# tqch/ddpm-torch

Measured on AMD Instinct MI355X. Metric: training imgs/s/GPU + 1000-step DDPM samples/s, CIFAR-10 UNet @1/2/4/8 MI355X, higher is better.
Workload: dtype bf16; 1 GPU; configs/cifar10.json UNet (35.7M params), full Trainer.step, B=128 per GPU, 32x32, T=1000, dropout 0.1, Adam+clip+EMA; global_batch=128, rccl_ranks=1, parallelism=dp1

## Files before the change

ddpm-torch_amd/csrc/build.py:

```python
import glob
import os
import subprocess
import sys

HERE = os.path.dirname(os.path.abspath(__file__))
SOURCES = ["gemm.hip", "wgrad.hip", "wgrad1x1.hip", "attention.hip", "attention_stream.hip", "pointwise.hip", "conv3x3.hip", "edgeconv.hip", "norm.hip", "elementwise.hip", "optim.hip", "probe.hip", "plan.hip", "toymlp.hip", "manifold.hip", "batch.hip", "ddim.hip", "guidance.hip"]
OUT = os.path.join(HERE, "libddpm_hip.so")
FLAGS = ["--offload-arch=gfx950", "-O3", "-std=c++17", "-munsafe-fp-atomics", "-fPIC"]


def _stale(target, deps):
    if not os.path.exists(target):
        return True
    t = os.path.getmtime(target)
    return any(os.path.getmtime(d) > t for d in deps)


def build(force=False, verbose=True):
    hipcc = os.environ.get("HIPCC", "/opt/rocm/bin/hipcc")
    hdrs = sorted(glob.glob(os.path.join(HERE, "*.h")))
    inc = os.path.join(HERE, "..", "..", "include")
    abi = [os.path.join(inc, "ddpm_hip.h"), os.path.join(inc, "ddpm_hip_debug.h")]
    objs = []
    procs = []
    for s in SOURCES:
        src, obj = os.path.join(HERE, s), os.path.join(HERE, s.replace(".hip", ".o"))
        objs.append(obj)
        if force or _stale(obj, [src, *hdrs, *abi]):
            cmd = [hipcc, *FLAGS, "-c", src, "-o", obj]
            if verbose:
                print(" ".join(cmd), flush=True)
            procs.append((cmd, subprocess.Popen(cmd)))
    for cmd, p in procs:
        if p.wait() != 0:
            raise RuntimeError("hipcc failed: " + " ".join(cmd))
    if force or procs or _stale(OUT, objs):
        cmd = [hipcc, "--offload-arch=gfx950", "-shared", "-fPIC", "-o", OUT, *objs]
        if verbose:
            print(" ".join(cmd), flush=True)
        subprocess.check_call(cmd)
    return OUT


if __name__ == "__main__":
    print(build(force="--force" in sys.argv))
```

ddpm-torch_amd/csrc/pointwise.hip:

```cpp
#include "common.h"
#include <string.h>
#include <stdlib.h>

namespace {

typedef float f32x4v __attribute__((ext_vector_type(4)));
typedef unsigned u32x2 __attribute__((ext_vector_type(2)));

struct PwArgs {
    const bf16_t* x; long long x_ld; unsigned x_extent;
    const bf16_t* w; unsigned w_extent;
    bf16_t* out; long long out_ld;
    const float* bias;
    const bf16_t* res; long long res_ld;
    int accumulate;
    int M, N, K, tiles_m, tiles_n, ksteps;
    int spread;
};

template <int TM, int TN>
__global__ __launch_bounds__(512, 2)
void pw_conv_kernel(PwArgs a) {
    constexpr int WN = TN / 64, WM = 8 / WN;
    constexpr int MJ = TM / (32 * WM);
    constexpr int XV = TM / 64;
    constexpr int WV = TN / 64;
    constexpr int PER = XV + WV;
    constexpr int RING = TM + TN == 256 ? 4 : 3;
    constexpr int XB = TM * 128, WB = TN * 128, STAGE = XB + WB;
    static_assert(TN == 128 || TN == 256, "channel tile");
    constexpr int BIAS_AT = RING * STAGE;
    static_assert(BIAS_AT + 4096 <= 160 * 1024, "LDS");
    extern __shared__ __attribute__((aligned(16))) char smem[];
    const int tid = threadIdx.x, lane = tid & 63;
    const int wave = __builtin_amdgcn_readfirstlane(tid >> 6);
    const int wn = wave / WM, wm = wave % WM;

    const __amdgpu_buffer_rsrc_t rx = buffer_rsrc(a.x, a.x_extent), rw = buffer_rsrc(a.w, a.w_extent);
    const __amdgpu_buffer_rsrc_t rb = buffer_rsrc(a.bias ? (const void*)a.bias : (const void*)a.w, a.bias ? (unsigned)(a.N * 4) : 0u);

    unsigned xoff[4], woff[4];
#pragma unroll
    for (int i = 0; i < XV; ++i) {
        const int v = tid + 512 * i, row = v >> 3, lc = (v & 7) ^ ((row >> 1) & 7);
        xoff[i] = (unsigned)(((long long)row * a.x_ld + lc * 8) * 2);
    }
#pragma unroll
    for (int i = 0; i < WV; ++i) {
        const int v = tid + 512 * i, row = v >> 3, lc = (v & 7) ^ ((row >> 1) & 7);
        woff[i] = (unsigned)(((long long)row * a.K + lc * 8) * 2);
    }
    const unsigned x_tile_bytes = (unsigned)((long long)TM * a.x_ld * 2), w_tile_bytes = (unsigned)((long long)TN * a.K * 2);

    const int units = a.spread ? a.tiles_m * a.tiles_n : a.tiles_m;
    const int my_units = units > (int)blockIdx.x ? (units - 1 - (int)blockIdx.x) / (int)gridDim.x + 1 : 0;
    const int total = my_units * (a.spread ? 1 : a.tiles_n) * a.ksteps;
    const int mt0 = a.spread ? (int)blockIdx.x / a.tiles_n : (int)blockIdx.x, nt0 = a.spread ? (int)blockIdx.x - mt0 * a.tiles_n : 0;
    int i_vt = blockIdx.x, i_mt = mt0, i_nt = nt0, i_ks = 0, i_q = 0, i_tile = 0;
    auto issue = [&]() {
        char* dst = smem + (i_q % RING) * STAGE;
        if (i_ks == 0) {
            if (wave == 0 && a.bias)
                LDS_DMA16(rb, smem + BIAS_AT + (i_tile & 3) * 1024, lane < TN / 4 ? (unsigned)((i_nt * TN + lane * 4) * 4) : BUF_OOB, 0);
            ++i_tile;
        }
        const unsigned xb = (unsigned)i_mt * x_tile_bytes + (unsigned)(i_ks * 128);
        const unsigned wb = (unsigned)i_nt * w_tile_bytes + (unsigned)(i_ks * 128);
#pragma unroll
        for (int i = 0; i < XV; ++i)
            LDS_DMA16(rx, dst + (wave * 64 + 512 * i) * 16, xb + xoff[i], 0);
#pragma unroll
        for (int i = 0; i < WV; ++i)
            LDS_DMA16(rw, dst + XB + (wave * 64 + 512 * i) * 16, wb + woff[i], 0);
        ++i_q;
        if (++i_ks == a.ksteps) {
            i_ks = 0;
            if (a.spread) { i_vt += gridDim.x; i_mt = i_vt / a.tiles_n; i_nt = i_vt - i_mt * a.tiles_n; }
            else if (++i_nt == a.tiles_n) { i_nt = 0; i_mt += gridDim.x; }
        }
    };

    f32x16 acc[2][MJ];
#pragma unroll
    for (int i = 0; i < 2; ++i)
#pragma unroll
        for (int j = 0; j < MJ; ++j) acc[i][j] = (f32x16)(0.f);

#pragma unroll
    for (int t = 0; t < RING - 1; ++t)
        if (t < total) issue();

    const int sw = (lane >> 5) ^ ((lane >> 1) & 7);
    int c_vt = blockIdx.x, c_mt = mt0, c_nt = nt0, c_ks = 0, c_tile = 0;
    constexpr int ST = 4 * MJ;
    int st_window = 0;
    for (int q = 0; q < total; ++q) {
        const int newer = min(RING - 2, total - 1 - q);
        if (st_window > 0) {
            --st_window;
            if (newer >= 2) wait_vm<2 * PER + ST>(); else if (newer == 1) wait_vm<PER + ST>(); else wait_vm<ST>();
        } else {
            if (newer >= 2) wait_vm<2 * PER>(); else if (newer == 1) wait_vm<PER>(); else wait_vm<0>();
        }
        __builtin_amdgcn_s_barrier();
        const bool last = c_ks + 1 == a.ksteps;
        u32x2 rv[MJ][2][4], ov[MJ][2][4];
        const bool pre = last && (a.res || a.accumulate);
        if (pre) {
            const int n0 = c_nt * TN + wn * 64, p0 = c_mt * TM + wm * (32 * MJ);
#pragma unroll
            for (int j = 0; j < MJ; ++j)
#pragma unroll
                for (int i = 0; i < 2; ++i)
#pragma unroll
                    for (int g = 0; g < 4; ++g) {
                        const int p = p0 + j * 32 + (lane & 31), n = n0 + i * 32 + 8 * g + 4 * (lane >> 5);
                        const bool ok = p < a.M && n < a.N;
                        rv[j][i][g] = (u32x2)(0u); ov[j][i][g] = (u32x2)(0u);
                        if (ok && a.res) asm volatile("global_load_dwordx2 %0, %1, off" : "=v"(rv[j][i][g]) : "v"(a.res + (long long)p * a.res_ld + n) : "memory");
                        if (ok && a.accumulate) asm volatile("global_load_dwordx2 %0, %1, off" : "=v"(ov[j][i][g]) : "v"(a.out + (long long)p * a.out_ld + n) : "memory");
                    }
        }
        const bool issued = i_q < total, bias_rides = issued && i_ks == 0 && wave == 0 && a.bias;
        if (issued) issue();
        const char* xs = smem + (q % RING) * STAGE;
        const char* ws = xs + XB;
#pragma unroll
        for (int kc = 0; kc < 4; ++kc) {
            u32x4 fw[2], fx[MJ];
#pragma unroll
            for (int i = 0; i < 2; ++i) fw[i] = *reinterpret_cast<const u32x4*>(ws + (wn * 64 + i * 32 + (lane & 31)) * 128 + (((2 * kc) ^ sw) << 4));
#pragma unroll
            for (int j = 0; j < MJ; ++j) fx[j] = *reinterpret_cast<const u32x4*>(xs + (wm * (32 * MJ) + j * 32 + (lane & 31)) * 128 + (((2 * kc) ^ sw) << 4));
#pragma unroll
            for (int i = 0; i < 2; ++i)
#pragma unroll
                for (int j = 0; j < MJ; ++j)
                    acc[i][j] = __builtin_amdgcn_mfma_f32_32x32x16_bf16(__builtin_bit_cast(bf16x8, fw[i]), __builtin_bit_cast(bf16x8, fx[j]), acc[i][j], 0, 0, 0);
        }
        asm volatile("s_waitcnt lgkmcnt(0)" ::: "memory");
        if (pre) {
            if (!issued) wait_vm<0>(); else if (bias_rides) wait_vm<PER + 1>(); else wait_vm<PER>();
            __builtin_amdgcn_sched_barrier(0);
        }
        if (last) {
            const int n0 = c_nt * TN + wn * 64, p0 = c_mt * TM + wm * (32 * MJ);
#pragma unroll
            for (int j = 0; j < MJ; ++j) {
                const int p = p0 + j * 32 + (lane & 31);
#pragma unroll
                for (int i = 0; i < 2; ++i) {
                    uint2 pk[4];
#pragma unroll
                    for (int g = 0; g < 4; ++g) {
                        const int n = n0 + i * 32 + 8 * g + 4 * (lane >> 5);
                        float v[4] = {acc[i][j][4 * g], acc[i][j][4 * g + 1], acc[i][j][4 * g + 2], acc[i][j][4 * g + 3]};
                        if (a.bias) {
                            f32x4v bv;
                            const unsigned baddr = lds_addr(smem + BIAS_AT + (c_tile & 3) * 1024 + (n - c_nt * TN) * 4);
                            asm volatile("ds_read_b128 %0, %1\n\ts_waitcnt lgkmcnt(0)" : "=v"(bv) : "v"(baddr) : "memory");
                            v[0] += bv.x; v[1] += bv.y; v[2] += bv.z; v[3] += bv.w;
                        }
                        if (a.res) {
                            const u32x2 r2 = rv[j][i][g];
                            v[0] += __uint_as_float(r2.x << 16); v[1] += __uint_as_float(r2.x & 0xffff0000u);
                            v[2] += __uint_as_float(r2.y << 16); v[3] += __uint_as_float(r2.y & 0xffff0000u);
                        }
                        if (a.accumulate) {
                            const u32x2 o2 = ov[j][i][g];
                            v[0] += __uint_as_float(o2.x << 16); v[1] += __uint_as_float(o2.x & 0xffff0000u);
                            v[2] += __uint_as_float(o2.y << 16); v[3] += __uint_as_float(o2.y & 0xffff0000u);
                        }
                        pk[g].x = pack_bf2(v[0], v[1]); pk[g].y = pack_bf2(v[2], v[3]);
                    }
#pragma unroll
                    for (int q2 = 0; q2 < 2; ++q2) {
                        const u32x2 sx = __builtin_amdgcn_permlane32_swap(pk[2 * q2].x, pk[2 * q2 + 1].x, false, false);
                        const u32x2 sy = __builtin_amdgcn_permlane32_swap(pk[2 * q2].y, pk[2 * q2 + 1].y, false, false);
                        const int n = n0 + i * 32 + 16 * q2 + 8 * (lane >> 5);
                        if (p < a.M && n < a.N) {
                            u32x4 o; o.x = sx.x; o.y = sy.x; o.z = sx.y; o.w = sy.y;
                            *reinterpret_cast<u32x4*>(a.out + (long long)p * a.out_ld + n) = o;
                        }
                    }
                }
            }
#pragma unroll
            for (int i = 0; i < 2; ++i)
#pragma unroll
                for (int j = 0; j < MJ; ++j) acc[i][j] = (f32x16)(0.f);
            st_window = (a.ksteps >= RING - 1 && c_nt * TN + wn * 64 + 64 <= a.N) ? RING - 1 : 0;
            c_ks = 0; ++c_tile;
            if (a.spread) { c_vt += gridDim.x; c_mt = c_vt / a.tiles_n; c_nt = c_vt - c_mt * a.tiles_n; }
            else if (++c_nt == a.tiles_n) { c_nt = 0; c_mt += gridDim.x; }
        } else ++c_ks;
    }
}

}

int ddpm_pointwise_launch(const void* x, long long x_ld, const void* w, void* y, long long y_ld, const float* bias, const void* residual,
                          long long res_ld, int accumulate, int M, int N, int K, int dry, void* stream) {
    constexpr int min_m = 8192;
    if (M < min_m || K % 64 || N % 8 || x_ld % 8 || y_ld % 8 || (residual && res_ld % 4)) return -1;
    if (!aligned16(x) || !aligned16(w) || !aligned16(y) || (residual && (((uintptr_t)residual) & 7)) || (bias && !aligned16(bias))) return -1;
    if ((long long)M * x_ld * 2 > BUF_OOB || (long long)N * K * 2 > BUF_OOB) return -1;
    if (dry) return DDPM_OK;
    PwArgs a; memset(&a, 0, sizeof(a));
    a.x = (const bf16_t*)x; a.x_ld = x_ld; a.x_extent = (unsigned)(((long long)(M - 1) * x_ld + K) * 2);
    a.w = (const bf16_t*)w; a.w_extent = (unsigned)((long long)N * K * 2);
    a.out = (bf16_t*)y; a.out_ld = y_ld; a.bias = bias; a.res = (const bf16_t*)residual; a.res_ld = res_ld; a.accumulate = accumulate;
    a.M = M; a.N = N; a.K = K; a.ksteps = K / 64;
    hipStream_t st = (hipStream_t)stream;
    const bool small_m = (M + 127) / 128 < 256;
    const bool wide = N >= 256;
    const bool big = (M + 255) / 256 >= 256;
    a.spread = small_m ? 1 : 0;
#define PW_LAUNCH(TM, TN, RINGV)                                                                                                  \
    do {                                                                                                                          \
        constexpr int LDS = RINGV * (TM * 128 + TN * 128) + 4096;                                                                 \
        static DevOnce attr_set;                                                                                                  \
        if (!attr_set) {                                                                                                          \
            if (hipFuncSetAttribute(reinterpret_cast<const void*>(&pw_conv_kernel<TM, TN>), hipFuncAttributeMaxDynamicSharedMemorySize, LDS) != hipSuccess) \
                return DDPM_ERR_LAUNCH;                                                                                           \
            attr_set = true;                                                                                                      \
        }                                                                                                                         \
        a.tiles_m = (M + TM - 1) / TM; a.tiles_n = (N + TN - 1) / TN;                                                             \
        const int units = a.spread ? a.tiles_m * a.tiles_n : a.tiles_m;                                                           \
        const int cus = ddpm_cu_budget(256);                                                                                      \
        const int grid = units < cus ? units : cus;                                                                               \
        hipLaunchKernelGGL((pw_conv_kernel<TM, TN>), dim3(grid), dim3(512), LDS, st, a);                                          \
    } while (0)
    if (wide) PW_LAUNCH(128, 256, 3); else if (big) PW_LAUNCH(256, 128, 3); else PW_LAUNCH(128, 128, 4);
#undef PW_LAUNCH
    return check_launch();
}
```

Before: 14430 imgs/s.

## Keep full 1x1-conv weight resident in LDS for pointwise GEMM when it fits

Adds a resident-weight variant of the pointwise (1x1 conv) kernel. When the whole weight matrix plus a 3- or 4-deep activation ring fits in 160KB of LDS, the weight is loaded once per block and only activation tiles are streamed. This removes repeated weight reloads per K-step and tile. The variant also switches residual and accumulate epilogue loads to 16-byte loads, reshuffled with permlane32 swaps. It costs larger LDS use per block, which lowers occupancy, plus an up-front weight-load prologue; the kernel moves into a shared header with a new compilation unit.

```diff
diff --git a/ddpm-torch_amd/csrc/build.py b/ddpm-torch_amd/csrc/build.py
--- a/ddpm-torch_amd/csrc/build.py
+++ b/ddpm-torch_amd/csrc/build.py
@@ -4,7 +4,7 @@
 import sys
 
 HERE = os.path.dirname(os.path.abspath(__file__))
-SOURCES = ["gemm.hip", "wgrad.hip", "wgrad1x1.hip", "attention.hip", "attention_stream.hip", "pointwise.hip", "conv3x3.hip", "edgeconv.hip", "norm.hip", "elementwise.hip", "optim.hip", "probe.hip", "plan.hip", "toymlp.hip", "manifold.hip", "batch.hip", "ddim.hip", "guidance.hip"]
+SOURCES = ["gemm.hip", "wgrad.hip", "wgrad1x1.hip", "attention.hip", "attention_stream.hip", "pointwise.hip", "pointwise_res.hip", "conv3x3.hip", "edgeconv.hip", "norm.hip", "elementwise.hip", "optim.hip", "probe.hip", "plan.hip", "toymlp.hip", "manifold.hip", "batch.hip", "ddim.hip", "guidance.hip"]
 OUT = os.path.join(HERE, "libddpm_hip.so")
 FLAGS = ["--offload-arch=gfx950", "-O3", "-std=c++17", "-munsafe-fp-atomics", "-fPIC"]
 
diff --git a/ddpm-torch_amd/csrc/pointwise.h b/ddpm-torch_amd/csrc/pointwise.h
--- /dev/null
+++ b/ddpm-torch_amd/csrc/pointwise.h
@@ -0,0 +1,264 @@
+#pragma once
+#include "common.h"
+
+struct PwArgs {
+    const bf16_t* x; long long x_ld; unsigned x_extent;
+    const bf16_t* w; unsigned w_extent;
+    bf16_t* out; long long out_ld;
+    const float* bias;
+    const bf16_t* res; long long res_ld;
+    int accumulate;
+    int M, N, K, tiles_m, tiles_n, ksteps;
+    int spread;
+    int nr;
+};
+
+#define PW_LAUNCH(KERNEL, TM, TN, LDS_MAX, LDS)                                                                                  \
+    do {                                                                                                                          \
+        static DevOnce attr_set;                                                                                                  \
+        if (!attr_set) {                                                                                                          \
+            if (hipFuncSetAttribute(reinterpret_cast<const void*>(&KERNEL), hipFuncAttributeMaxDynamicSharedMemorySize, LDS_MAX) != hipSuccess) \
+                return DDPM_ERR_LAUNCH;                                                                                           \
+            attr_set = true;                                                                                                      \
+        }                                                                                                                         \
+        a.tiles_m = (M + TM - 1) / TM; a.tiles_n = (N + TN - 1) / TN;                                                             \
+        const int units = a.spread ? a.tiles_m * a.tiles_n : a.tiles_m;                                                           \
+        const int cus = ddpm_cu_budget(256);                                                                                      \
+        const int grid = units < cus ? units : cus;                                                                               \
+        hipLaunchKernelGGL((KERNEL), dim3(grid), dim3(512), LDS, st, a);                                                          \
+    } while (0)
+int ddpm_pointwise_resident_launch(PwArgs& a, int ring, int lds, hipStream_t st);
+
+namespace {
+
+typedef float f32x4v __attribute__((ext_vector_type(4)));
+typedef unsigned u32x2 __attribute__((ext_vector_type(2)));
+
+
+template <int TM, int TN, int RING, bool RES>
+__global__ __launch_bounds__(512, 2)
+void pw_conv_kernel(PwArgs a) {
+    constexpr int WN = TN / 64, WM = 8 / WN;
+    constexpr int MJ = TM / (32 * WM);
+    constexpr int XV = TM / 64;
+    constexpr int WV = TN / 64;
+    constexpr int PER = RES ? XV : XV + WV;
+    constexpr bool R16 = RES;
+    constexpr int XB = TM * 128, WB = TN * 128, STAGE = RES ? XB : XB + WB;
+    static_assert(TN == 128 || TN == 256, "channel tile");
+    static_assert(RING == 3 || RING == 4, "the waits below know 1 or 2 newer stages; 4 bias slots cover a ring of 4 at one K-step per tile");
+    constexpr int BIAS_AT = RING * STAGE;
+    constexpr int W_AT = BIAS_AT + 4096;
+    static_assert(W_AT <= 160 * 1024, "LDS");
+    extern __shared__ __attribute__((aligned(16))) char smem[];
+    const int tid = threadIdx.x, lane = tid & 63;
+    const int wave = __builtin_amdgcn_readfirstlane(tid >> 6);
+    const int wn = wave / WM, wm = wave % WM;
+
+    const __amdgpu_buffer_rsrc_t rx = buffer_rsrc(a.x, a.x_extent), rw = buffer_rsrc(a.w, a.w_extent);
+    const __amdgpu_buffer_rsrc_t rb = buffer_rsrc(a.bias ? (const void*)a.bias : (const void*)a.w, a.bias ? (unsigned)(a.N * 4) : 0u);
+
+    unsigned xoff[4], woff[4] = {0u, 0u, 0u, 0u};
+#pragma unroll
+    for (int i = 0; i < XV; ++i) {
+        const int v = tid + 512 * i, row = v >> 3, lc = (v & 7) ^ ((row >> 1) & 7);
+        xoff[i] = (unsigned)(((long long)row * a.x_ld + lc * 8) * 2);
+    }
+    if constexpr (!RES) {
+#pragma unroll
+        for (int i = 0; i < WV; ++i) {
+            const int v = tid + 512 * i, row = v >> 3, lc = (v & 7) ^ ((row >> 1) & 7);
+            woff[i] = (unsigned)(((long long)row * a.K + lc * 8) * 2);
+        }
+    }
+    const unsigned x_tile_bytes = (unsigned)((long long)TM * a.x_ld * 2), w_tile_bytes = (unsigned)((long long)TN * a.K * 2);
+
+    const int units = a.spread ? a.tiles_m * a.tiles_n : a.tiles_m;
+    const int my_units = units > (int)blockIdx.x ? (units - 1 - (int)blockIdx.x) / (int)gridDim.x + 1 : 0;
+    const int total = my_units * (a.spread ? 1 : a.tiles_n) * a.ksteps;
+    const int mt0 = a.spread ? (int)blockIdx.x / a.tiles_n : (int)blockIdx.x, nt0 = a.spread ? (int)blockIdx.x - mt0 * a.tiles_n : 0;
+    int i_vt = blockIdx.x, i_mt = mt0, i_nt = nt0, i_ks = 0, i_q = 0, i_tile = 0;
+    auto issue = [&]() {
+        char* dst = smem + (i_q % RING) * STAGE;
+        if (i_ks == 0) {
+            if (wave == 0 && a.bias)
+                LDS_DMA16(rb, smem + BIAS_AT + (i_tile & 3) * 1024, lane < TN / 4 ? (unsigned)((i_nt * TN + lane * 4) * 4) : BUF_OOB, 0);
+            ++i_tile;
+        }
+        const unsigned xb = (unsigned)i_mt * x_tile_bytes + (unsigned)(i_ks * 128);
+        const unsigned wb = (unsigned)i_nt * w_tile_bytes + (unsigned)(i_ks * 128);
+#pragma unroll
+        for (int i = 0; i < XV; ++i)
+            LDS_DMA16(rx, dst + (wave * 64 + 512 * i) * 16, xb + xoff[i], 0);
+        if constexpr (!RES) {
+#pragma unroll
+            for (int i = 0; i < WV; ++i)
+                LDS_DMA16(rw, dst + XB + (wave * 64 + 512 * i) * 16, wb + woff[i], 0);
+        }
+        ++i_q;
+        if (++i_ks == a.ksteps) {
+            i_ks = 0;
+            if (a.spread) { i_vt += gridDim.x; i_mt = i_vt / a.tiles_n; i_nt = i_vt - i_mt * a.tiles_n; }
+            else if (++i_nt == a.tiles_n) { i_nt = 0; i_mt += gridDim.x; }
+        }
+    };
+
+    f32x16 acc[2][MJ];
+#pragma unroll
+    for (int i = 0; i < 2; ++i)
+#pragma unroll
+        for (int j = 0; j < MJ; ++j) acc[i][j] = (f32x16)(0.f);
+
+    if constexpr (RES) {
+        int g_lo = 0, g_hi = a.nr >> 6;
+        if (a.spread && my_units <= 1) { g_lo = nt0 * (TN / 64); g_hi = min(g_lo + TN / 64, g_hi); }
+        if (total > 0)
+            for (int ks = 0; ks < a.ksteps; ++ks)
+                for (int g = g_lo; g < g_hi; ++g) {
+                    const int row = g * 64 + (tid >> 3), lc = (tid & 7) ^ ((row >> 1) & 7);
+                    LDS_DMA16(rw, smem + W_AT + ((ks * a.nr + g * 64) * 8 + wave * 64) * 16, (unsigned)((row * a.K + ks * 64 + lc * 8) * 2), 0);
+                }
+    }
+#pragma unroll
+    for (int t = 0; t < RING - 1; ++t)
+        if (t < total) issue();
+
+    const int sw = (lane >> 5) ^ ((lane >> 1) & 7);
+    int c_vt = blockIdx.x, c_mt = mt0, c_nt = nt0, c_ks = 0, c_tile = 0;
+    constexpr int ST = 4 * MJ;
+    int st_window = 0;
+    for (int q = 0; q < total; ++q) {
+        const int newer = min(RING - 2, total - 1 - q);
+        if (st_window > 0) {
+            --st_window;
+            if (newer >= 2) wait_vm<2 * PER + ST>(); else if (newer == 1) wait_vm<PER + ST>(); else wait_vm<ST>();
+        } else {
+            if (newer >= 2) wait_vm<2 * PER>(); else if (newer == 1) wait_vm<PER>(); else wait_vm<0>();
+        }
+        __builtin_amdgcn_s_barrier();
+        const bool last = c_ks + 1 == a.ksteps;
+        u32x2 rv[MJ][2][4], ov[MJ][2][4];
+        u32x4 rw4[MJ][2][2], ow4[MJ][2][2];
+        const bool pre = last && (a.res || a.accumulate);
+        if (pre) {
+            const int n0 = c_nt * TN + wn * 64, p0 = c_mt * TM + wm * (32 * MJ);
+#pragma unroll
+            for (int j = 0; j < MJ; ++j)
+#pragma unroll
+                for (int i = 0; i < 2; ++i)
+                    if constexpr (R16) {
+#pragma unroll
+                        for (int h = 0; h < 2; ++h) {
+                            const int p = p0 + j * 32 + (lane & 31), n = n0 + i * 32 + 16 * h + 8 * (lane >> 5);
+                            const bool ok = p < a.M && n < a.N;
+                            rw4[j][i][h] = (u32x4)(0u); ow4[j][i][h] = (u32x4)(0u);
+                            if (ok && a.res) asm volatile("global_load_dwordx4 %0, %1, off" : "=v"(rw4[j][i][h]) : "v"(a.res + (long long)p * a.res_ld + n) : "memory");
+                            if (ok && a.accumulate) asm volatile("global_load_dwordx4 %0, %1, off" : "=v"(ow4[j][i][h]) : "v"(a.out + (long long)p * a.out_ld + n) : "memory");
+                        }
+                    } else {
+#pragma unroll
+                        for (int g = 0; g < 4; ++g) {
+                            const int p = p0 + j * 32 + (lane & 31), n = n0 + i * 32 + 8 * g + 4 * (lane >> 5);
+                            const bool ok = p < a.M && n < a.N;
+                            rv[j][i][g] = (u32x2)(0u); ov[j][i][g] = (u32x2)(0u);
+                            if (ok && a.res) asm volatile("global_load_dwordx2 %0, %1, off" : "=v"(rv[j][i][g]) : "v"(a.res + (long long)p * a.res_ld + n) : "memory");
+                            if (ok && a.accumulate) asm volatile("global_load_dwordx2 %0, %1, off" : "=v"(ov[j][i][g]) : "v"(a.out + (long long)p * a.out_ld + n) : "memory");
+                        }
+                    }
+        }
+        const bool issued = i_q < total, bias_rides = issued && i_ks == 0 && wave == 0 && a.bias;
+        if (issued) issue();
+        const char* xs = smem + (q % RING) * STAGE;
+        const char* ws = RES ? smem + W_AT + (c_ks * a.nr + min(c_nt * TN + wn * 64, a.nr - 64)) * 128 : xs + XB + wn * 64 * 128;
+#pragma unroll
+        for (int kc = 0; kc < 4; ++kc) {
+            u32x4 fw[2], fx[MJ];
+#pragma unroll
+            for (int i = 0; i < 2; ++i) fw[i] = *reinterpret_cast<const u32x4*>(ws + (i * 32 + (lane & 31)) * 128 + (((2 * kc) ^ sw) << 4));
+#pragma unroll
+            for (int j = 0; j < MJ; ++j) fx[j] = *reinterpret_cast<const u32x4*>(xs + (wm * (32 * MJ) + j * 32 + (lane & 31)) * 128 + (((2 * kc) ^ sw) << 4));
+#pragma unroll
+            for (int i = 0; i < 2; ++i)
+#pragma unroll
+                for (int j = 0; j < MJ; ++j)
+                    acc[i][j] = __builtin_amdgcn_mfma_f32_32x32x16_bf16(__builtin_bit_cast(bf16x8, fw[i]), __builtin_bit_cast(bf16x8, fx[j]), acc[i][j], 0, 0, 0);
+        }
+        asm volatile("s_waitcnt lgkmcnt(0)" ::: "memory");
+        if (pre) {
+            if (!issued) wait_vm<0>(); else if (bias_rides) wait_vm<PER + 1>(); else wait_vm<PER>();
+            __builtin_amdgcn_sched_barrier(0);
+        }
+        if (last) {
+            const int n0 = c_nt * TN + wn * 64, p0 = c_mt * TM + wm * (32 * MJ);
+#pragma unroll
+            for (int j = 0; j < MJ; ++j) {
+                const int p = p0 + j * 32 + (lane & 31);
+#pragma unroll
+                for (int i = 0; i < 2; ++i) {
+                    uint2 pk[4];
+                    if constexpr (R16) {
+                        if (a.res) {
+#pragma unroll
+                            for (int h = 0; h < 2; ++h) {
+                                const u32x2 sx = __builtin_amdgcn_permlane32_swap(rw4[j][i][h].x, rw4[j][i][h].z, false, false);
+                                const u32x2 sy = __builtin_amdgcn_permlane32_swap(rw4[j][i][h].y, rw4[j][i][h].w, false, false);
+                                rv[j][i][2 * h].x = sx.x; rv[j][i][2 * h].y = sy.x; rv[j][i][2 * h + 1].x = sx.y; rv[j][i][2 * h + 1].y = sy.y;
+                            }
+                        }
+                        if (a.accumulate) {
+#pragma unroll
+                            for (int h = 0; h < 2; ++h) {
+                                const u32x2 sx = __builtin_amdgcn_permlane32_swap(ow4[j][i][h].x, ow4[j][i][h].z, false, false);
+                                const u32x2 sy = __builtin_amdgcn_permlane32_swap(ow4[j][i][h].y, ow4[j][i][h].w, false, false);
+                                ov[j][i][2 * h].x = sx.x; ov[j][i][2 * h].y = sy.x; ov[j][i][2 * h + 1].x = sx.y; ov[j][i][2 * h + 1].y = sy.y;
+                            }
+                        }
+                    }
+#pragma unroll
+                    for (int g = 0; g < 4; ++g) {
+                        const int n = n0 + i * 32 + 8 * g + 4 * (lane >> 5);
+                        float v[4] = {acc[i][j][4 * g], acc[i][j][4 * g + 1], acc[i][j][4 * g + 2], acc[i][j][4 * g + 3]};
+                        if (a.bias) {
+                            f32x4v bv;
+                            const unsigned baddr = lds_addr(smem + BIAS_AT + (c_tile & 3) * 1024 + (n - c_nt * TN) * 4);
+                            asm volatile("ds_read_b128 %0, %1\n\ts_waitcnt lgkmcnt(0)" : "=v"(bv) : "v"(baddr) : "memory");
+                            v[0] += bv.x; v[1] += bv.y; v[2] += bv.z; v[3] += bv.w;
+                        }
+                        if (a.res) {
+                            const u32x2 r2 = rv[j][i][g];
+                            v[0] += __uint_as_float(r2.x << 16); v[1] += __uint_as_float(r2.x & 0xffff0000u);
+                            v[2] += __uint_as_float(r2.y << 16); v[3] += __uint_as_float(r2.y & 0xffff0000u);
+                        }
+                        if (a.accumulate) {
+                            const u32x2 o2 = ov[j][i][g];
+                            v[0] += __uint_as_float(o2.x << 16); v[1] += __uint_as_float(o2.x & 0xffff0000u);
+                            v[2] += __uint_as_float(o2.y << 16); v[3] += __uint_as_float(o2.y & 0xffff0000u);
+                        }
+                        pk[g].x = pack_bf2(v[0], v[1]); pk[g].y = pack_bf2(v[2], v[3]);
+                    }
+#pragma unroll
+                    for (int q2 = 0; q2 < 2; ++q2) {
+                        const u32x2 sx = __builtin_amdgcn_permlane32_swap(pk[2 * q2].x, pk[2 * q2 + 1].x, false, false);
+                        const u32x2 sy = __builtin_amdgcn_permlane32_swap(pk[2 * q2].y, pk[2 * q2 + 1].y, false, false);
+                        const int n = n0 + i * 32 + 16 * q2 + 8 * (lane >> 5);
+                        if (p < a.M && n < a.N) {
+                            u32x4 o; o.x = sx.x; o.y = sy.x; o.z = sx.y; o.w = sy.y;
+                            *reinterpret_cast<u32x4*>(a.out + (long long)p * a.out_ld + n) = o;
+                        }
+                    }
+                }
+            }
+#pragma unroll
+            for (int i = 0; i < 2; ++i)
+#pragma unroll
+                for (int j = 0; j < MJ; ++j) acc[i][j] = (f32x16)(0.f);
+            st_window = (a.ksteps >= RING - 1 && c_nt * TN + wn * 64 + 64 <= a.N) ? RING - 1 : 0;
+            c_ks = 0; ++c_tile;
+            if (a.spread) { c_vt += gridDim.x; c_mt = c_vt / a.tiles_n; c_nt = c_vt - c_mt * a.tiles_n; }
+            else if (++c_nt == a.tiles_n) { c_nt = 0; c_mt += gridDim.x; }
+        } else ++c_ks;
+    }
+}
+
+
+}
diff --git a/ddpm-torch_amd/csrc/pointwise.hip b/ddpm-torch_amd/csrc/pointwise.hip
--- a/ddpm-torch_amd/csrc/pointwise.hip
+++ b/ddpm-torch_amd/csrc/pointwise.hip
@@ -1,203 +1,7 @@
-#include "common.h"
+#include "pointwise.h"
 #include <string.h>
 #include <stdlib.h>
 
-namespace {
-
-typedef float f32x4v __attribute__((ext_vector_type(4)));
-typedef unsigned u32x2 __attribute__((ext_vector_type(2)));
-
-struct PwArgs {
-    const bf16_t* x; long long x_ld; unsigned x_extent;
-    const bf16_t* w; unsigned w_extent;
-    bf16_t* out; long long out_ld;
-    const float* bias;
-    const bf16_t* res; long long res_ld;
-    int accumulate;
-    int M, N, K, tiles_m, tiles_n, ksteps;
-    int spread;
-};
-
-template <int TM, int TN>
-__global__ __launch_bounds__(512, 2)
-void pw_conv_kernel(PwArgs a) {
-    constexpr int WN = TN / 64, WM = 8 / WN;
-    constexpr int MJ = TM / (32 * WM);
-    constexpr int XV = TM / 64;
-    constexpr int WV = TN / 64;
-    constexpr int PER = XV + WV;
-    constexpr int RING = TM + TN == 256 ? 4 : 3;
-    constexpr int XB = TM * 128, WB = TN * 128, STAGE = XB + WB;
-    static_assert(TN == 128 || TN == 256, "channel tile");
-    constexpr int BIAS_AT = RING * STAGE;
-    static_assert(BIAS_AT + 4096 <= 160 * 1024, "LDS");
-    extern __shared__ __attribute__((aligned(16))) char smem[];
-    const int tid = threadIdx.x, lane = tid & 63;
-    const int wave = __builtin_amdgcn_readfirstlane(tid >> 6);
-    const int wn = wave / WM, wm = wave % WM;
-
-    const __amdgpu_buffer_rsrc_t rx = buffer_rsrc(a.x, a.x_extent), rw = buffer_rsrc(a.w, a.w_extent);
-    const __amdgpu_buffer_rsrc_t rb = buffer_rsrc(a.bias ? (const void*)a.bias : (const void*)a.w, a.bias ? (unsigned)(a.N * 4) : 0u);
-
-    unsigned xoff[4], woff[4];
-#pragma unroll
-    for (int i = 0; i < XV; ++i) {
-        const int v = tid + 512 * i, row = v >> 3, lc = (v & 7) ^ ((row >> 1) & 7);
-        xoff[i] = (unsigned)(((long long)row * a.x_ld + lc * 8) * 2);
-    }
-#pragma unroll
-    for (int i = 0; i < WV; ++i) {
-        const int v = tid + 512 * i, row = v >> 3, lc = (v & 7) ^ ((row >> 1) & 7);
-        woff[i] = (unsigned)(((long long)row * a.K + lc * 8) * 2);
-    }
-    const unsigned x_tile_bytes = (unsigned)((long long)TM * a.x_ld * 2), w_tile_bytes = (unsigned)((long long)TN * a.K * 2);
-
-    const int units = a.spread ? a.tiles_m * a.tiles_n : a.tiles_m;
-    const int my_units = units > (int)blockIdx.x ? (units - 1 - (int)blockIdx.x) / (int)gridDim.x + 1 : 0;
-    const int total = my_units * (a.spread ? 1 : a.tiles_n) * a.ksteps;
-    const int mt0 = a.spread ? (int)blockIdx.x / a.tiles_n : (int)blockIdx.x, nt0 = a.spread ? (int)blockIdx.x - mt0 * a.tiles_n : 0;
-    int i_vt = blockIdx.x, i_mt = mt0, i_nt = nt0, i_ks = 0, i_q = 0, i_tile = 0;
-    auto issue = [&]() {
-        char* dst = smem + (i_q % RING) * STAGE;
-        if (i_ks == 0) {
-            if (wave == 0 && a.bias)
-                LDS_DMA16(rb, smem + BIAS_AT + (i_tile & 3) * 1024, lane < TN / 4 ? (unsigned)((i_nt * TN + lane * 4) * 4) : BUF_OOB, 0);
-            ++i_tile;
-        }
-        const unsigned xb = (unsigned)i_mt * x_tile_bytes + (unsigned)(i_ks * 128);
-        const unsigned wb = (unsigned)i_nt * w_tile_bytes + (unsigned)(i_ks * 128);
-#pragma unroll
-        for (int i = 0; i < XV; ++i)
-            LDS_DMA16(rx, dst + (wave * 64 + 512 * i) * 16, xb + xoff[i], 0);
-#pragma unroll
-        for (int i = 0; i < WV; ++i)
-            LDS_DMA16(rw, dst + XB + (wave * 64 + 512 * i) * 16, wb + woff[i], 0);
-        ++i_q;
-        if (++i_ks == a.ksteps) {
-            i_ks = 0;
-            if (a.spread) { i_vt += gridDim.x; i_mt = i_vt / a.tiles_n; i_nt = i_vt - i_mt * a.tiles_n; }
-            else if (++i_nt == a.tiles_n) { i_nt = 0; i_mt += gridDim.x; }
-        }
-    };
-
-    f32x16 acc[2][MJ];
-#pragma unroll
-    for (int i = 0; i < 2; ++i)
-#pragma unroll
-        for (int j = 0; j < MJ; ++j) acc[i][j] = (f32x16)(0.f);
-
-#pragma unroll
-    for (int t = 0; t < RING - 1; ++t)
-        if (t < total) issue();
-
-    const int sw = (lane >> 5) ^ ((lane >> 1) & 7);
-    int c_vt = blockIdx.x, c_mt = mt0, c_nt = nt0, c_ks = 0, c_tile = 0;
-    constexpr int ST = 4 * MJ;
-    int st_window = 0;
-    for (int q = 0; q < total; ++q) {
-        const int newer = min(RING - 2, total - 1 - q);
-        if (st_window > 0) {
-            --st_window;
-            if (newer >= 2) wait_vm<2 * PER + ST>(); else if (newer == 1) wait_vm<PER + ST>(); else wait_vm<ST>();
-        } else {
-            if (newer >= 2) wait_vm<2 * PER>(); else if (newer == 1) wait_vm<PER>(); else wait_vm<0>();
-        }
-        __builtin_amdgcn_s_barrier();
-        const bool last = c_ks + 1 == a.ksteps;
-        u32x2 rv[MJ][2][4], ov[MJ][2][4];
-        const bool pre = last && (a.res || a.accumulate);
-        if (pre) {
-            const int n0 = c_nt * TN + wn * 64, p0 = c_mt * TM + wm * (32 * MJ);
-#pragma unroll
-            for (int j = 0; j < MJ; ++j)
-#pragma unroll
-                for (int i = 0; i < 2; ++i)
-#pragma unroll
-                    for (int g = 0; g < 4; ++g) {
-                        const int p = p0 + j * 32 + (lane & 31), n = n0 + i * 32 + 8 * g + 4 * (lane >> 5);
-                        const bool ok = p < a.M && n < a.N;
-                        rv[j][i][g] = (u32x2)(0u); ov[j][i][g] = (u32x2)(0u);
-                        if (ok && a.res) asm volatile("global_load_dwordx2 %0, %1, off" : "=v"(rv[j][i][g]) : "v"(a.res + (long long)p * a.res_ld + n) : "memory");
-                        if (ok && a.accumulate) asm volatile("global_load_dwordx2 %0, %1, off" : "=v"(ov[j][i][g]) : "v"(a.out + (long long)p * a.out_ld + n) : "memory");
-                    }
-        }
-        const bool issued = i_q < total, bias_rides = issued && i_ks == 0 && wave == 0 && a.bias;
-        if (issued) issue();
-        const char* xs = smem + (q % RING) * STAGE;
-        const char* ws = xs + XB;
-#pragma unroll
-        for (int kc = 0; kc < 4; ++kc) {
-            u32x4 fw[2], fx[MJ];
-#pragma unroll
-            for (int i = 0; i < 2; ++i) fw[i] = *reinterpret_cast<const u32x4*>(ws + (wn * 64 + i * 32 + (lane & 31)) * 128 + (((2 * kc) ^ sw) << 4));
-#pragma unroll
-            for (int j = 0; j < MJ; ++j) fx[j] = *reinterpret_cast<const u32x4*>(xs + (wm * (32 * MJ) + j * 32 + (lane & 31)) * 128 + (((2 * kc) ^ sw) << 4));
-#pragma unroll
-            for (int i = 0; i < 2; ++i)
-#pragma unroll
-                for (int j = 0; j < MJ; ++j)
-                    acc[i][j] = __builtin_amdgcn_mfma_f32_32x32x16_bf16(__builtin_bit_cast(bf16x8, fw[i]), __builtin_bit_cast(bf16x8, fx[j]), acc[i][j], 0, 0, 0);
-        }
-        asm volatile("s_waitcnt lgkmcnt(0)" ::: "memory");
-        if (pre) {
-            if (!issued) wait_vm<0>(); else if (bias_rides) wait_vm<PER + 1>(); else wait_vm<PER>();
-            __builtin_amdgcn_sched_barrier(0);
-        }
-        if (last) {
-            const int n0 = c_nt * TN + wn * 64, p0 = c_mt * TM + wm * (32 * MJ);
-#pragma unroll
-            for (int j = 0; j < MJ; ++j) {
-                const int p = p0 + j * 32 + (lane & 31);
-#pragma unroll
-                for (int i = 0; i < 2; ++i) {
-                    uint2 pk[4];
-#pragma unroll
-                    for (int g = 0; g < 4; ++g) {
-                        const int n = n0 + i * 32 + 8 * g + 4 * (lane >> 5);
-                        float v[4] = {acc[i][j][4 * g], acc[i][j][4 * g + 1], acc[i][j][4 * g + 2], acc[i][j][4 * g + 3]};
-                        if (a.bias) {
-                            f32x4v bv;
-                            const unsigned baddr = lds_addr(smem + BIAS_AT + (c_tile & 3) * 1024 + (n - c_nt * TN) * 4);
-                            asm volatile("ds_read_b128 %0, %1\n\ts_waitcnt lgkmcnt(0)" : "=v"(bv) : "v"(baddr) : "memory");
-                            v[0] += bv.x; v[1] += bv.y; v[2] += bv.z; v[3] += bv.w;
-                        }
-                        if (a.res) {
-                            const u32x2 r2 = rv[j][i][g];
-                            v[0] += __uint_as_float(r2.x << 16); v[1] += __uint_as_float(r2.x & 0xffff0000u);
-                            v[2] += __uint_as_float(r2.y << 16); v[3] += __uint_as_float(r2.y & 0xffff0000u);
-                        }
-                        if (a.accumulate) {
-                            const u32x2 o2 = ov[j][i][g];
-                            v[0] += __uint_as_float(o2.x << 16); v[1] += __uint_as_float(o2.x & 0xffff0000u);
-                            v[2] += __uint_as_float(o2.y << 16); v[3] += __uint_as_float(o2.y & 0xffff0000u);
-                        }
-                        pk[g].x = pack_bf2(v[0], v[1]); pk[g].y = pack_bf2(v[2], v[3]);
-                    }
-#pragma unroll
-                    for (int q2 = 0; q2 < 2; ++q2) {
-                        const u32x2 sx = __builtin_amdgcn_permlane32_swap(pk[2 * q2].x, pk[2 * q2 + 1].x, false, false);
-                        const u32x2 sy = __builtin_amdgcn_permlane32_swap(pk[2 * q2].y, pk[2 * q2 + 1].y, false, false);
-                        const int n = n0 + i * 32 + 16 * q2 + 8 * (lane >> 5);
-                        if (p < a.M && n < a.N) {
-                            u32x4 o; o.x = sx.x; o.y = sy.x; o.z = sx.y; o.w = sy.y;
-                            *reinterpret_cast<u32x4*>(a.out + (long long)p * a.out_ld + n) = o;
-                        }
-                    }
-                }
-            }
-#pragma unroll
-            for (int i = 0; i < 2; ++i)
-#pragma unroll
-                for (int j = 0; j < MJ; ++j) acc[i][j] = (f32x16)(0.f);
-            st_window = (a.ksteps >= RING - 1 && c_nt * TN + wn * 64 + 64 <= a.N) ? RING - 1 : 0;
-            c_ks = 0; ++c_tile;
-            if (a.spread) { c_vt += gridDim.x; c_mt = c_vt / a.tiles_n; c_nt = c_vt - c_mt * a.tiles_n; }
-            else if (++c_nt == a.tiles_n) { c_nt = 0; c_mt += gridDim.x; }
-        } else ++c_ks;
-    }
-}
-
-}
 
 int ddpm_pointwise_launch(const void* x, long long x_ld, const void* w, void* y, long long y_ld, const float* bias, const void* residual,
                           long long res_ld, int accumulate, int M, int N, int K, int dry, void* stream) {
@@ -216,22 +20,13 @@
     const bool wide = N >= 256;
     const bool big = (M + 255) / 256 >= 256;
     a.spread = small_m ? 1 : 0;
-#define PW_LAUNCH(TM, TN, RINGV)                                                                                                  \
-    do {                                                                                                                          \
-        constexpr int LDS = RINGV * (TM * 128 + TN * 128) + 4096;                                                                 \
-        static DevOnce attr_set;                                                                                                  \
-        if (!attr_set) {                                                                                                          \
-            if (hipFuncSetAttribute(reinterpret_cast<const void*>(&pw_conv_kernel<TM, TN>), hipFuncAttributeMaxDynamicSharedMemorySize, LDS) != hipSuccess) \
-                return DDPM_ERR_LAUNCH;                                                                                           \
-            attr_set = true;                                                                                                      \
-        }                                                                                                                         \
-        a.tiles_m = (M + TM - 1) / TM; a.tiles_n = (N + TN - 1) / TN;                                                             \
-        const int units = a.spread ? a.tiles_m * a.tiles_n : a.tiles_m;                                                           \
-        const int cus = ddpm_cu_budget(256);                                                                                      \
-        const int grid = units < cus ? units : cus;                                                                               \
-        hipLaunchKernelGGL((pw_conv_kernel<TM, TN>), dim3(grid), dim3(512), LDS, st, a);                                          \
-    } while (0)
-    if (wide) PW_LAUNCH(128, 256, 3); else if (big) PW_LAUNCH(256, 128, 3); else PW_LAUNCH(128, 128, 4);
-#undef PW_LAUNCH
+    a.nr = (N + 63) / 64 * 64;
+    const long long w_lds = (long long)a.nr * K * 2;
+    constexpr long long lds_cap = 160 * 1024, res_stage = 128 * 128;
+    const int res_ring = w_lds + 4 * res_stage + 4096 <= lds_cap ? 4 : w_lds + 3 * res_stage + 4096 <= lds_cap ? 3 : 0;
+#define PW_STREAM(TM, TN, RINGV) PW_LAUNCH((pw_conv_kernel<TM, TN, RINGV, false>), TM, TN, RINGV * (TM * 128 + TN * 128) + 4096, RINGV * (TM * 128 + TN * 128) + 4096)
+    if (res_ring) return ddpm_pointwise_resident_launch(a, res_ring, res_ring * (int)res_stage + 4096 + (int)w_lds, st);
+    if (wide) PW_STREAM(128, 256, 3); else if (big) PW_STREAM(256, 128, 3); else PW_STREAM(128, 128, 4);
+#undef PW_STREAM
     return check_launch();
 }
diff --git a/ddpm-torch_amd/csrc/pointwise_res.hip b/ddpm-torch_amd/csrc/pointwise_res.hip
--- /dev/null
+++ b/ddpm-torch_amd/csrc/pointwise_res.hip
@@ -0,0 +1,12 @@
+#include "pointwise.h"
+
+int ddpm_pointwise_resident_launch(PwArgs& a, int ring, int lds, hipStream_t st) {
+    const int M = a.M, N = a.N;
+    constexpr int lds_cap = 160 * 1024;
+    if ((ring != 3 && ring != 4) || lds > lds_cap) return DDPM_ERR_LAUNCH;
+#define PW_RESIDENT(TN, RINGV) PW_LAUNCH((pw_conv_kernel<128, TN, RINGV, true>), 128, TN, lds_cap, lds)
+    if (N >= 256) { if (ring == 4) PW_RESIDENT(256, 4); else PW_RESIDENT(256, 3); }
+    else { if (ring == 4) PW_RESIDENT(128, 4); else PW_RESIDENT(128, 3); }
+#undef PW_RESIDENT
+    return check_launch();
+}
```

Measured after the change: 14500 imgs/s, median of 6. Within noise of the previous version (+0.5%).
